# SudhirNikam/cobrix

Hardware: AMD Instinct MI355X
Metric: decoded input GB/s + records/s, fixed-len COMP-3 mix, 1-8 MI355X; % HBM peak (higher is better)
Workload: dtype u8; 1 GPU; SYN200: fixed-length 200-byte EBCDIC records, numeric mix (COMP, COMP-3, zoned DISPLAY overpunch, IBM COMP-2, cp037 X(18)) -- BASELINE config C2; records_per_gpu=50000000, input_bytes_per_gpu=10000000000, job_input_bytes=10000000000, output_columns=28, parallelism=dp1, string_layout=Arrow string views (16 B views + long payloads, one pass), occurs_layout=Arrow lists (present elements only), inputs_resident_in_hbm=True

## Files before the change

cobrix_amd/csrc/cbx_capi.hip:

```cpp
#include <hip/hip_runtime.h>

#include <algorithm>
#include <cstdio>
#include <cstring>
#include <functional>
#include <string>
#include <vector>

#include "cbx_kernels.hip"
#include "cbx_select.h"
#include "cbx_text.h"
#include "cbx_hier.h"
#include "cbx_walk.h"
#include "cbx_chain.h"
#include "cbx_filter.h"
#include "cbx_aggregate.h"
#include "cbx_group.h"
#include "cbx_topn.h"
#include "cbx_keyset.h"
#include "cbx_gather.h"

using namespace cbx;

static thread_local std::string g_err;
// ... 44 lines not shown
    bool view = false;
    bool packed = false;
    std::vector<int32_t> segid_cols;
    std::vector<ListOp> lops;
    ListOp* d_lops = nullptr;
    int32_t* d_list_len = nullptr;  int64_t list_len_cap = 0;
    int32_t* d_list_flag = nullptr; int64_t list_flag_cap = 0;
    Field* d_fields = nullptr;
    DeferSeq* d_defer = nullptr;
    uint64_t* d_defer_bits = nullptr;
    int64_t defer_bits_cap = 0;
    cbx_array* d_arrays = nullptr;
    cbx_segment_map* d_segmap = nullptr;
    uint32_t* d_lut = nullptr;
    DevColumn* d_cols = nullptr;
    std::vector<DevColumn> h_cols;
    std::vector<NumCall> h_ncall;
    std::vector<StrCall> h_scall;
    NumCall* d_ncall = nullptr;
    StrCall* d_scall = nullptr;
    size_t ncall_cap = 0, scall_cap = 0;
    std::vector<int32_t> seq_field, seq_slot;
    std::vector<int64_t> seq_tile_cap;
    std::vector<SeqCall> h_seqcall;
    std::vector<int64_t> h_seq_scratch;
    SeqCall* d_seqcall = nullptr;
    uint32_t* d_str_tot = nullptr;  int64_t str_tot_cap = 0;
    int64_t* d_str_excl = nullptr;  int64_t str_excl_cap = 0;
    int64_t* d_block_sums = nullptr; int64_t block_sums_cap = 0;
    uint32_t* d_local = nullptr;    int64_t local_cap = 0;
    uint8_t* d_scratch = nullptr;   int64_t scratch_cap = 0;
    uint64_t* d_stamps = nullptr;
    int64_t jit_min = 262144;
    bool jit_tried[4 * kPre + 5] = {};
    hipFunction_t jit_fn[4 * kPre + 5] = {};
    bool jit_coop[4 * kPre + 5] = {};
    int rec_extent = 0;
    std::string jit_error;
    int last_kind = 0;
    cbx_launch_info last_info{};
    cbx_walk_info last_walk{};
    int32_t* d_status = nullptr;
    int num_cus = 256;
    bool walk = false;
    int32_t walk_root = 0, walk_var = 0, walk_n_handlers = 0, walk_depth = 1, walk_max_rec = 0;
    cbx_walk_node* d_wnodes = nullptr;
    std::vector<cbx_walk_node> h_wnodes;
    std::vector<cbx_walk_array> h_warr;
    bool walk_jit_tried = false;
    hipFunction_t walk_jit_fn = nullptr;
    bool chain_jit_tried = false;
    hipFunction_t chain_jit_fn[5] = {};
    bool last_chain_jit = false;
    cbx_walk_array* d_warr = nullptr;
    cbx_walk_handler* d_whand = nullptr;
    int64_t* d_wslot_base = nullptr;
    int64_t* d_wtile_bytes = nullptr;
    const int64_t* d_rec_base = nullptr;
    const int32_t* d_odo = nullptr;
    int64_t odo_pitch = 0;
    const int64_t* d_dep_seed = nullptr;
    int64_t seed_pitch = 0;
    int32_t seed_root = -1;
    int64_t n_str_slots = 0;
    uint32_t* d_wcursor = nullptr; int64_t wcursor_cap = 0;
    int64_t* d_wvbase = nullptr;
    int32_t* d_wvcol = nullptr;
    int32_t* d_wvslot = nullptr;
    int32_t n_vslots = 0;
// ... 509 lines not shown

static int jit_pro(const cbx_plan* P) { return (P->opts.has_segments ? 1 : 0) | (P->harrays.empty() ? 0 : 2); }

static int launch(cbx_plan* P, const CallShape& c, const cbx_column* columns, int mode, hipStream_t st) {
    const int64_t n_tiles = (c.n_rec + kWave - 1) / kWave;
    KernelArgs a{};
    uintptr_t addr = (uintptr_t)c.data;
    a.base_shift = (int64_t)(addr & 15);
    a.data = (const uint8_t*)(addr & ~(uintptr_t)15);
    a.data_len = c.data_len + a.base_shift;
    a.rec_off = c.rec_off;
    a.rec_len = c.rec_len;
    a.n_rec = c.n_rec;
    a.n_tiles = n_tiles;
    a.pitch = n_tiles * kWave;
    a.stride = c.stride;
    a.start_off = c.start_off;
    a.first_record_id = c.first_record_id;
    a.rec_id_base = P->d_rec_base;
    a.rec_id = c.rec_id;
    a.rec_seg = c.rec_seg;
    a.odo_count = P->d_odo;
    a.odo_pitch = P->odo_pitch;
    a.file_id = c.file_id >= 0 ? c.file_id : P->opts.file_id;
    a.mode = mode;
    a.str_view = str_layout_of(P);
    const int sdw = c.stride / 4;
    const bool contig = !c.rec_off && P->contig_ok && c.stride > 0 && c.stride % 4 == 0 && a.base_shift % 4 == 0 &&
                        contig_kp(sdw) <= kPre;
    a.contig = contig ? 1 : 0;
    const int span_ext = c.start_off + P->rec_extent;
    const int span_kp = (int)std::min<int64_t>(kPre, ((int64_t)kWave * (span_ext + 8) + 32 + 1023) / 1024);
    hipFunction_t span_fn = nullptr;
    if (c.rec_off && !c.rec_id && !c.rec_seg && P->contig_ok && mode == 0 && P->jit_min >= 0 && c.n_rec >= P->jit_min &&
        (int64_t)kWave * span_ext <= 16 * 1024 && !getenv("CBX_NO_SPAN")) {
        const int k = kPre + 1 + span_kp;
        if (!P->jit_tried[k]) {
            P->jit_tried[k] = true;
            P->jit_fn[k] = jit_get(jit_source(true, span_kp, jit_pro(P), str_layout_of(P), P->cset.win, P->cset.nops, P->cset.batches,
                                              P->cset.sops, true), &P->jit_error);
        }
        span_fn = P->jit_fn[k];
    }
    const bool span = span_fn != nullptr;
    const cbx_plan::OpSet& S = (contig || span) ? P->cset : P->wset;
    if (span) {
        a.span_ext = span_ext;
        const int nch = (P->rec_extent + 15 + 15) >> 4;
        a.span_pitch = 16 * nch + 4;
        a.lds_rows = kGuard + std::max(span_kp * 1024 + 64, kWave * a.span_pitch) + kGuard;
    } else if (contig) {
        a.stride_dw = sdw;
        const int g = std::__gcd(sdw, 32);
        a.cpitch = 4 * ((g >= 4 || (g == 2 && getenv("CBX_PAD_ROWS"))) ? ((sdw & 1) ? sdw : sdw + 1) : sdw);
        a.inv_stride_dw = 1.0f / (float)sdw;
        a.lds_rows = kGuard + kWave * a.cpitch + 16 + kGuard;
    } else {
        a.lds_rows = kGuard + kWave * std::max(P->max_pitch, 16) + kGuard;
    }
    a.windows = (const CBX_CONST Window*)S.d_win;
    a.n_windows = (int)S.win.size();
    a.nops = (const CBX_CONST NumOp*)S.d_nops;
    a.batches = (const CBX_CONST Batch*)S.d_batches;
    a.sops = (const CBX_CONST StrOp*)S.d_sops;
    a.gops = (const CBX_CONST GenOp*)S.d_gops;
    a.lds_rows = (a.lds_rows + 15) & ~15;
    a.lds_counts = ((int)P->harrays.size() * kWave * 4 + 15) & ~15;
    a.str_stage = S.max_str_items > 0 ? (P->view && mode == 0 && P->view_staged ? std::max(P->str_stage, 16 * kWave) : P->str_stage) : 0;
    const int lds_base = a.lds_rows + a.lds_counts + a.str_stage;
    auto lds_blocks = [](int per_wave) {
        return (160 * 1024) / (kLutLds + kWavesPerBlock * ((per_wave + 15) & ~15));
    };
    const bool lane_dump = a.str_stage > 0 && lds_blocks(lds_base + 4 * kWave) >= lds_blocks(lds_base + 16);
    a.dump_stride = lane_dump ? 4 : 0;
    a.lds_wave = (lds_base + (lane_dump ? 4 * kWave : 16) + 15) & ~15;
    a.fields = (const CBX_CONST Field*)P->d_fields;
    a.arrays = (const CBX_CONST cbx_array*)P->d_arrays;
    a.n_arrays = (int)P->harrays.size();
    a.seg_col = P->seg_col;
    a.segmap = P->opts.has_segments ? (const CBX_CONST cbx_segment_map*)P->d_segmap : nullptr;
    a.lut = P->d_lut;
    a.cols = (const CBX_CONST DevColumn*)P->d_cols;
    a.n_seq = P->n_seq;
    a.status = P->d_status;
#ifdef CBX_STAMPS
    if (!P->d_stamps) {
        HIP_CHECK(hipMalloc((void**)&P->d_stamps, 8 * sizeof(uint64_t)));
        HIP_CHECK(hipMemset(P->d_stamps, 0, 8 * sizeof(uint64_t)));
// ... 101 lines not shown
            HIP_CHECK(hipMalloc((void**)&P->d_ncall, sizeof(NumCall) * P->h_ncall.size()));
            P->ncall_cap = P->h_ncall.size();
        }
        if (P->h_scall.size() > P->scall_cap) {
            HIP_CHECK(hipStreamSynchronize(st));
            (void)hipFree(P->d_scall);
            P->d_scall = nullptr;
            HIP_CHECK(hipMalloc((void**)&P->d_scall, sizeof(StrCall) * P->h_scall.size()));
            P->scall_cap = P->h_scall.size();
        }
        if (!P->h_ncall.empty())
            HIP_CHECK(hipMemcpyAsync(P->d_ncall, P->h_ncall.data(), sizeof(NumCall) * P->h_ncall.size(), hipMemcpyHostToDevice, st));
        if (!P->h_scall.empty())
            HIP_CHECK(hipMemcpyAsync(P->d_scall, P->h_scall.data(), sizeof(StrCall) * P->h_scall.size(), hipMemcpyHostToDevice, st));
    }
    a.ncall = (const CBX_CONST NumCall*)P->d_ncall;
    a.scall = (const CBX_CONST StrCall*)P->d_scall;
    int r;
    if (P->n_seq > 0 && (r = grow(&P->d_str_tot, &P->str_tot_cap, (int64_t)P->n_seq * n_tiles, st))) return r;
    a.str_tot = P->d_str_tot;
    const bool lists = mode == 0 && !P->lops.empty();
    if (lists && ((r = grow(&P->d_list_len, &P->list_len_cap, (int64_t)P->harrays.size() * a.pitch, st)) ||
                  (r = grow(&P->d_list_flag, &P->list_flag_cap, n_tiles, st))))
        return r;
    a.list_len = P->d_list_len;
    a.list_flag = P->d_list_flag;
    const int n_defer = n_defer_seq;
    a.defer_bits = P->d_defer_bits;
    const size_t lds_own = kLutLds + (size_t)kWavesPerBlock * a.lds_wave;
    if (lds_own > 160 * 1024) return fail(CBX_E_UNSUPPORTED, "record window does not fit in LDS");
    hipFunction_t jfn = span_fn;
    int jk = -1;
    if (!span && mode == 0 && P->jit_min >= 0 && c.n_rec >= P->jit_min) {
        const int k = contig ? contig_kp(sdw) : 0;
        if (!P->jit_tried[k]) {
            P->jit_tried[k] = true;
            size_t elems = S.sops.size();
            for (const NumOp& o : S.nops) elems += o.run > 1 ? o.run : 1;
            if (elems > (size_t)kJitMaxOps || S.win.size() > (size_t)kJitMaxWindows)
                P->jit_error = "layout has " + std::to_string(elems) + " elements in " + std::to_string(S.win.size()) +
                               " windows, above the specialised-kernel limits (" + std::to_string(kJitMaxOps) + ", " +
                               std::to_string(kJitMaxWindows) + ")";
            else {
                CoopSplit cs;
                P->jit_coop[k] = jit_coop_of(contig, span, jit_pro(P), str_layout_of(P), S.win, S.nops, S.batches, S.sops, false, &cs);
                P->jit_fn[k] = jit_get(jit_source(contig, k, jit_pro(P), str_layout_of(P), S.win, S.nops, S.batches, S.sops, false), &P->jit_error);
            }
        }
        jfn = P->jit_fn[k];
        jk = k;
    }
    P->last_kind = jfn ? 1 : 0;
    const bool coop = jfn && jk >= 0 && P->jit_coop[jk];
    const size_t lds = coop ? kLutLds + (size_t)a.lds_rows + (size_t)kWavesPerBlock * (a.lds_wave - a.lds_rows) : lds_own;
    if (lds > 160 * 1024) return fail(CBX_E_UNSUPPORTED, "record window does not fit in LDS");
    int blocks_per_cu = (int)std::max<size_t>(1, std::min<size_t>(16, (160 * 1024) / lds));
    int occ = 0;
    const hipError_t oe = jfn ? hipModuleOccupancyMaxActiveBlocksPerMultiprocessor(&occ, jfn, kWave * kWavesPerBlock, lds)
                              : hipOccupancyMaxActiveBlocksPerMultiprocessor(&occ, decode_kernel, kWave * kWavesPerBlock, lds);
    if (oe == hipSuccess && occ > 0) blocks_per_cu = std::min(blocks_per_cu, occ);
    if (!coop && contig && S.sops.size() >= S.nops.size() && S.sops.size() > 0) blocks_per_cu = std::min(blocks_per_cu, 4);
    if (const char* e = getenv("CBX_MAX_BLOCKS_PER_CU")) blocks_per_cu = std::max(1, std::min(blocks_per_cu, atoi(e)));
    const bool piped = P->pipe_peer && mode == 0 && P->packed && P->n_seq > 0;
    if (piped && P->pipe_decode_bpc > 0) blocks_per_cu = std::min(blocks_per_cu, P->pipe_decode_bpc);
    const int64_t blocks_needed = coop ? n_tiles : (n_tiles + kWavesPerBlock - 1) / kWavesPerBlock;
    const int64_t grid = std::min<int64_t>(blocks_needed, (int64_t)P->num_cus * blocks_per_cu);
    const bool prof = P->profiling && mode == 0;
    cbx_plan::CallEvents ce{{nullptr, nullptr, nullptr}};
    if (piped && P->pipe_peer->pipe_done) HIP_CHECK(hipStreamWaitEvent(st, P->pipe_peer->pipe_done, 0));
    if (prof) {
        for (auto& e : ce.e) if (!(e = take_event(P))) return fail(CBX_E_HIP, "hipEventCreate failed");
        HIP_CHECK(hipEventRecord(ce.e[0], st));
    }
    hipFunction_t cfn = nullptr;
    int ck = 0;
    if (mode == 0 && P->packed && P->n_seq > 0 && (contig || span) && P->jit_min >= 0 && c.n_rec >= P->jit_min) {
        const int kp = contig ? contig_kp(sdw) : span_kp;
        const int k = (contig ? 2 : 3) * (kPre + 1) + kp;
        if (!P->jit_tried[k]) {
            P->jit_tried[k] = true;
            std::string err;
            CoopSplit cs;
            P->jit_coop[k] = jit_coop_of(true, span, jit_pro(P), 2, S.win, S.nops, S.batches, S.sops, true, &cs);
            P->jit_fn[k] = jit_get(jit_source(true, kp, jit_pro(P), 2, S.win, S.nops, S.batches, S.sops, span, true),
                                   &err, "cbx_jit_count");
        }
        cfn = P->jit_fn[k];
        ck = k;
    }
    if (mode == 0 && P->packed && P->n_seq > 0 && !cfn && !contig) {
        const int kind = P->last_kind;
        if ((r = launch(P, c, columns, 1, st))) return r;
        P->last_kind = kind;
        if (piped) HIP_CHECK(hipEventRecord(P->pipe_done, st));
    } else if (mode == 0 && P->packed && P->n_seq > 0) {
        KernelArgs ac = a;
        ac.mode = 1;
        size_t clds = lds_own;
        const bool ccoop = cfn && P->jit_coop[ck];
        if (cfn) {
            ac.lds_wave = (a.lds_rows + a.lds_counts + 16 + 15) & ~15;
            clds = 1024 + kLutLds + (ccoop ? (size_t)a.lds_rows + (size_t)kWavesPerBlock * (ac.lds_wave - a.lds_rows)
                                           : (size_t)kWavesPerBlock * ac.lds_wave);
        }
        int cocc = 0;
        const hipError_t ce2 = cfn ? hipModuleOccupancyMaxActiveBlocksPerMultiprocessor(&cocc, cfn, kWave * kWavesPerBlock, clds)
                                   : hipOccupancyMaxActiveBlocksPerMultiprocessor(&cocc, decode_kernel, kWave * kWavesPerBlock, clds);
        int cbpc = (int)std::max<size_t>(1, std::min<size_t>(16, (160 * 1024) / clds));
        if (ce2 == hipSuccess && cocc > 0) cbpc = std::min(cbpc, cocc);
        if (const char* e = getenv("CBX_MAX_BLOCKS_PER_CU")) cbpc = std::max(1, std::min(cbpc, atoi(e)));
        if (piped && P->pipe_count_bpc > 0) cbpc = std::min(cbpc, P->pipe_count_bpc);
        const int64_t cneeded = ccoop ? n_tiles : (n_tiles + kWavesPerBlock - 1) / kWavesPerBlock;
        const int64_t cgrid = std::min<int64_t>(cneeded, (int64_t)P->num_cus * cbpc);
        if (cfn) {
            void* kargs[] = {&ac};
            HIP_CHECK(hipModuleLaunchKernel(cfn, (unsigned)cgrid, 1, 1, kWave * kWavesPerBlock, 1, 1, (unsigned)clds, st, kargs, nullptr));
        } else {
            hipLaunchKernelGGL(decode_kernel, dim3((unsigned)cgrid), dim3(kWave * kWavesPerBlock), clds, st, ac);
            HIP_CHECK(hipGetLastError());
        }
        if ((r = string_scan(P, n_tiles, st))) return r;
        if (piped) HIP_CHECK(hipEventRecord(P->pipe_done, st));
    }
    if (mode == 0) {
        cbx_launch_info li{};
        li.kind = P->last_kind;
        li.staging = span ? 2 : contig ? 1 : 0;
        li.coop = coop ? 1 : 0;
        li.kp = contig ? contig_kp(sdw) : span ? span_kp : 0;
        li.padded_rows = contig && a.cpitch != c.stride ? 1 : 0;
        li.n_windows = (int32_t)S.win.size();
        for (const Window& w : S.win)
            if (w.global && (w.nop_end > w.nop_begin || w.sop_end > w.sop_begin)) li.global_window = 1;
        li.count_kernel = !(P->packed && P->n_seq > 0) ? 0 : cfn ? 1 : 2;
        li.base_shift = (int32_t)a.base_shift;
        li.grid = grid;
        li.blocks_needed = blocks_needed;
        P->last_info = li;
    }
    if (jfn) {
        void* kargs[] = {&a};
        HIP_CHECK(hipModuleLaunchKernel(jfn, (unsigned)grid, 1, 1, kWave * kWavesPerBlock, 1, 1, (unsigned)lds, st, kargs, nullptr));
    } else {
        hipLaunchKernelGGL(decode_kernel, dim3((unsigned)grid), dim3(kWave * kWavesPerBlock), lds, st, a);
        HIP_CHECK(hipGetLastError());
    }
    if (lists) {
        const int64_t lgrid = std::min<int64_t>((n_tiles + kListWaves - 1) / kListWaves, (int64_t)P->num_cus * 8);
        const size_t llds = kListWaves * 2 * (2 * kGuard + kListStage);
        hipFunction_t lfn = nullptr;
        if (P->jit_min >= 0 && c.n_rec >= P->jit_min) {
            const int k = 4 * (kPre + 1);
            if (!P->jit_tried[k]) {
                P->jit_tried[k] = true;
                const std::string src = jit_list_source(P->lops);
                std::string err;
                if (!src.empty()) P->jit_fn[k] = jit_get(src, &err, "cbx_jit_list");
            }
            lfn = P->jit_fn[k];
        }
        const CBX_CONST ListOp* d_lops = (const CBX_CONST ListOp*)P->d_lops;
        int32_t n_lops = (int32_t)P->lops.size();
        if (lfn) {
            void* kargs[] = {&a, &d_lops, &n_lops};
            HIP_CHECK(hipModuleLaunchKernel(lfn, (unsigned)lgrid, 1, 1, kWave * kListWaves, 1, 1, (unsigned)llds, st, kargs, nullptr));
        } else {
            hipLaunchKernelGGL(list_kernel<false>, dim3((unsigned)lgrid), dim3(kWave * kListWaves), llds, st, a, d_lops, n_lops);
        }
// ... 2527 lines not shown
```

cobrix_amd/csrc/cbx_device.h:

```cpp
#pragma once
#ifndef __HIPCC_RTC__
#include <hip/hip_runtime.h>
#endif

#include "cbx_internal.h"

#ifndef CBX_DIAG
#define CBX_DIAG 0
#endif

namespace cbx {

__device__ __forceinline__ uint32_t wave_excl_scan32(uint32_t x, int lane, uint32_t& total) {
    uint32_t v = x;
    v += (uint32_t)__builtin_amdgcn_update_dpp(0, (int)v, 0x111, 0xF, 0xF, true);
    v += (uint32_t)__builtin_amdgcn_update_dpp(0, (int)v, 0x112, 0xF, 0xF, true);
    v += (uint32_t)__builtin_amdgcn_update_dpp(0, (int)v, 0x114, 0xF, 0xF, true);
    v += (uint32_t)__builtin_amdgcn_update_dpp(0, (int)v, 0x118, 0xF, 0xF, true);
    const uint32_t r0 = (uint32_t)__builtin_amdgcn_readlane((int)v, 15);
    const uint32_t r1 = (uint32_t)__builtin_amdgcn_readlane((int)v, 31);
    const uint32_t r2 = (uint32_t)__builtin_amdgcn_readlane((int)v, 47);
    const uint32_t r3 = (uint32_t)__builtin_amdgcn_readlane((int)v, 63);
    const int row = lane >> 4;
    v += (row >= 1 ? r0 : 0u) + (row >= 2 ? r1 : 0u) + (row >= 3 ? r2 : 0u);
// ... 1452 lines not shown

__device__ __forceinline__ ContigSpan contig_span(const KernelArgs& a, int64_t tile) {
    ContigSpan sp;
    const int64_t t0b = a.base_shift + tile * kWave * (int64_t)a.stride;
    const int64_t left = a.n_rec - tile * kWave;
    const int nrec_tile = left < kWave ? (left > 0 ? (int)left : 0) : kWave;
    sp.a0 = t0b & ~(int64_t)15;
    sp.mis_dw = (int)((t0b - sp.a0) >> 2);
    sp.span_dw = nrec_tile * a.stride_dw;
    sp.nch = (sp.mis_dw + sp.span_dw + 3) >> 2;
    return sp;
}

template <int KP>
__device__ __forceinline__ void contig_issue(const KernelArgs& a, const ContigSpan& sp, int lane, uint4 (&buf)[KP]) {
    int64_t left = (a.data_len - sp.a0 + 3) & ~(int64_t)3;
    left = left < 0 ? 0 : (left > (1 << 20) ? (1 << 20) : left);
    const uint64_t base = (uint64_t)(a.data + sp.a0);
    const uint32_t lo = __builtin_amdgcn_readfirstlane((uint32_t)base);
    const uint32_t hi = __builtin_amdgcn_readfirstlane((uint32_t)(base >> 32));
    const int nbytes = __builtin_amdgcn_readfirstlane((int)left);
    const int nch = __builtin_amdgcn_readfirstlane(sp.nch);
    void* bp = (void*)(((uint64_t)hi << 32) | lo);
    const __amdgpu_buffer_rsrc_t rs = __builtin_amdgcn_make_buffer_rsrc(bp, (short)0, nbytes, 0x00020000);
#pragma unroll
    for (int u = 0; u < KP; u++) {
        const int c = u * kWave + lane;
        const int off = c < nch ? 16 * c : 0x7ffffff0;
        const auto v = __builtin_amdgcn_raw_buffer_load_b128(rs, off, 0, kStageCpol);
        buf[u] = make_uint4(v[0], v[1], v[2], v[3]);
    }
}

__device__ __forceinline__ void contig_put(const KernelArgs& a, const ContigSpan& sp, int c, uint4 v, uint8_t* s_img) {
    if (a.cpitch == 4 * a.stride_dw) {
        *(uint4*)(s_img + 16 * c) = v;
        return;
    }
    uint32_t* img32 = (uint32_t*)s_img;
    const uint32_t wv[4] = {v.x, v.y, v.z, v.w};
#pragma unroll
    for (int k = 0; k < 4; k++) {
        const int d = 4 * c + k - sp.mis_dw;
        if (d >= 0 && d < sp.span_dw) {
            const int r = (int)(((float)d + 0.5f) * a.inv_stride_dw);
            img32[d + sp.mis_dw + r] = wv[k];
        }
    }
}

template <int KP>
__device__ __forceinline__ void contig_store(const KernelArgs& a, const ContigSpan& sp, int lane, const uint4 (&buf)[KP],
                                             uint8_t* s_img) {
    asm volatile("" : "+v"(lane));
#pragma unroll
    for (int u = 0; u < KP; u++) {
        const int c = u * kWave + lane;
        if (u * kWave < sp.nch && c < sp.nch) contig_put(a, sp, c, buf[u], s_img);
    }
}

__device__ __forceinline__ uint32_t stage_window(const KernelArgs& a, const Window& w, const TileCtx& t,
                                                 uint8_t* s_img, int lane) {
    const int W = w.hi - w.lo;
    const int pitch = w.pitch;
    const int nch = (W + 15 + 15) >> 4;
    const float inv_nch = 1.0f / (float)nch;
    const int64_t my_g = t.base + a.start_off + w.lo;
// ... 187 lines not shown

template <int KP, int kPro, bool kLate, typename Body>
__device__ __forceinline__ void contig_loop(const KernelArgs& a, const WaveLds& l, int64_t tile, int64_t tstep,
                                            int lane, Body body) {
    uint4 buf[KP];
    tile = first_tile<Body>(tile);
    if (tile < a.n_tiles) contig_issue<KP>(a, contig_span(a, tile), lane, buf);
    Stamps st;
    st.init();
    while (tile < a.n_tiles) {
        const ContigSpan sp = contig_span(a, tile);
        contig_store<KP>(a, sp, lane, buf, l.img);
        wave_sync_lds();
        st.mark(0);
        const int64_t next = next_tile<Body>(tile, tstep);
        body.begin(tile);
        if (!kLate) contig_issue<KP>(a, contig_span(a, next), lane, buf);
        st.mark(1);
        TileCtx t = tile_ctx<false>(a, tile, lane);
        const uint32_t rec0 = (uint32_t)(lane * a.cpitch + 4 * sp.mis_dw);
        tile_prologue<false, (kPro & 1) != 0, (kPro & 2) != 0>(a, t, l.img + rec0, lane, l.lut, l.cnt);
        st.mark(2);
        body.pre(a, t, (const uint8_t*)l.img, rec0 + (uint32_t)a.start_off, l, lane, st);
        if (kLate) contig_issue<KP>(a, contig_span(a, next), lane, buf);
        body.post(a, t, (const uint8_t*)l.img, rec0 + (uint32_t)a.start_off, l, lane, st);
        run_end(a, body, tile, lane);
        wave_sync_lds();
        st.mark(5);
        tile = next;
    }
    st.flush(a, lane);
}

template <int KP>
__device__ __forceinline__ void coop_issue(const KernelArgs& a, const ContigSpan& sp, int wid, int lane,
                                           uint4 (&buf)[(KP + kWavesPerBlock - 1) / kWavesPerBlock]) {
    constexpr int KH = (KP + kWavesPerBlock - 1) / kWavesPerBlock;
    int64_t left = a.data_len - sp.a0;
    left = left < 0 ? 0 : (left > (1 << 20) ? (1 << 20) : left);
    const uint64_t base = (uint64_t)(a.data + sp.a0);
    const uint32_t lo = __builtin_amdgcn_readfirstlane((uint32_t)base);
    const uint32_t hi = __builtin_amdgcn_readfirstlane((uint32_t)(base >> 32));
    const int nbytes = __builtin_amdgcn_readfirstlane((int)left);
    const int nch = __builtin_amdgcn_readfirstlane(sp.nch);
    void* bp = (void*)(((uint64_t)hi << 32) | lo);
    const __amdgpu_buffer_rsrc_t rs = __builtin_amdgcn_make_buffer_rsrc(bp, (short)0, nbytes, 0x00020000);
#pragma unroll
    for (int v = 0; v < KH; v++) {
        const int c = (v * kWavesPerBlock + wid) * kWave + lane;
        const int off = c < nch ? 16 * c : 0x7ffffff0;
        const auto x = __builtin_amdgcn_raw_buffer_load_b128(rs, off, 0, kStageCpol);
        buf[v] = make_uint4(x[0], x[1], x[2], x[3]);
    }
}

template <int KP>
__device__ __forceinline__ void coop_put(const KernelArgs& a, const ContigSpan& sp, int wid, int lane,
                                         const uint4 (&buf)[(KP + kWavesPerBlock - 1) / kWavesPerBlock], uint8_t* s_img) {
    constexpr int KH = (KP + kWavesPerBlock - 1) / kWavesPerBlock;
    int ln = lane;
    asm volatile("" : "+v"(ln));
#pragma unroll
    for (int v = 0; v < KH; v++) {
        const int c = (v * kWavesPerBlock + wid) * kWave + ln;
        if (c < sp.nch) contig_put(a, sp, c, buf[v], s_img);
    }
}

template <int KP, int kW, typename Body>
__device__ __forceinline__ void coop_loop(const KernelArgs& a, const WaveLds& l, int64_t tile, int64_t tstep,
                                          int lane, Body body) {
    constexpr int KH = (KP + kWavesPerBlock - 1) / kWavesPerBlock;
    uint4 buf[KH];
    constexpr int wid = kW;
    body.wid = wid;
#ifndef CBX_NO_COOP_PRIO
    if (wid == 1) __builtin_amdgcn_s_setprio(1);
#endif
    tile = first_tile<Body>(tile);
    if (tile >= a.n_tiles) return;
    coop_issue<KP>(a, contig_span(a, tile), wid, lane, buf);
    coop_put<KP>(a, contig_span(a, tile), wid, lane, buf, l.img);
    Stamps st;
    st.init();
    while (true) {
        __syncthreads();
        st.mark(0);
        const ContigSpan sp = contig_span(a, tile);
        const int64_t next = next_tile<Body>(tile, tstep);
        body.begin(tile);
        coop_issue<KP>(a, contig_span(a, next), wid, lane, buf);
        st.mark(1);
        TileCtx t = tile_ctx<false>(a, tile, lane);
        const uint32_t rec0 = (uint32_t)(lane * a.cpitch + 4 * sp.mis_dw);
        st.mark(2);
        body.template part<kW>(a, t, (const uint8_t*)l.img, rec0 + (uint32_t)a.start_off, l, lane, st);
        run_end(a, body, tile, lane);
        __syncthreads();
        st.mark(5);
        tile = next;
        if (tile >= a.n_tiles) break;
        coop_put<KP>(a, contig_span(a, tile), wid, lane, buf, l.img);
    }
    st.flush(a, lane);
}

__device__ __forceinline__ void span_recs(const KernelArgs& a, int64_t tile, int lane, int64_t& off, int32_t& len) {
    const int64_t r = tile * kWave + lane;
    const int64_t rc = r < a.n_rec ? r : a.n_rec - 1;
    const int64_t o = a.rec_off[rc];
    const int32_t l = a.rec_len[rc];
    off = a.base_shift + o;
    len = r < a.n_rec ? l : 0;
}

__device__ __forceinline__ int64_t wave_min64(int64_t v) {
#pragma unroll
    for (int m = 1; m < kWave; m <<= 1) {
        const int64_t o = __shfl_xor(v, m, kWave);
        v = o < v ? o : v;
    }
    return v;
}
__device__ __forceinline__ int64_t wave_max64(int64_t v) {
#pragma unroll
    for (int m = 1; m < kWave; m <<= 1) {
        const int64_t o = __shfl_xor(v, m, kWave);
        v = o > v ? o : v;
    }
    return v;
}

template <int KP>
__device__ __forceinline__ ContigSpan span_of(const KernelArgs& a, int64_t tile, int64_t off, int32_t len) {
    const int64_t lo = wave_min64(off);
// ... 81 lines not shown
```

cobrix_amd/csrc/cbx_jit.h:

```cpp
#pragma once
#include <hip/hiprtc.h>

#include <algorithm>
#include <cstdlib>
#include <map>
#include <mutex>
#include <sstream>
#include <string>
#include <utility>
#include <vector>

#include "cbx_jit_src.inc"

namespace cbx {

constexpr int kJitMaxStrUnroll = 16;

static std::string jit_u64(uint64_t v) {
    std::ostringstream o;
    o << "0x" << std::hex << v << "ull";
    return o.str();
}

static void jit_numop(std::ostringstream& o, const NumOp& n) {
// ... 179 lines not shown
    out->sop_mid = m_best <= ns ? sb + m_best : se;
    out->nop_mid = m_best <= ns ? 0 : m_best - ns;
    const int nnum = (int)nops.size();
    int n_defer = 0;
    for (const NumOp& op : nops) n_defer = std::max(n_defer, op.defer + 1);
    out->own[0] = out->own[1] = 0;
    for (int i = 0; i < nnum && n_words > 0; i++) {
        const int w = i < out->nop_mid ? 0 : 1;
        out->own[w] |= 1ull << i;
        if (nops[i].defer >= 0) out->own[w] |= 1ull << (nnum + nops[i].defer);
    }
    for (int i = sb; i < se && i - sb < n_str_words; i++) out->own[i < out->sop_mid ? 0 : 1] |= 1ull << (nnum + n_defer + i);
    return true;
}

static int jit_words(int layout, const std::vector<NumOp>& nops, const std::vector<Batch>& batches,
                     const std::vector<StrOp>& sops, bool span, bool count, int* n_str_words) {
    int n_defer = 0;
    bool runs = false;
    for (const NumOp& op : nops) n_defer = std::max(n_defer, op.defer + 1);
    for (const Batch& b : batches) runs |= b.runs != 0;
    *n_str_words = layout == 1 && getenv("CBX_STR_VWORDS") ? (int)sops.size() : 0;
    return (count || runs || span || getenv("CBX_NO_VWORDS")) ? 0 : (int)nops.size() + n_defer + *n_str_words;
}

static bool jit_coop_of(bool contig, bool span, int pro, int layout, const std::vector<Window>& win, const std::vector<NumOp>& nops,
                        const std::vector<Batch>& batches, const std::vector<StrOp>& sops, bool count, CoopSplit* out) {
    int nsw = 0;
    const int nw = contig ? jit_words(layout, nops, batches, sops, span, count, &nsw) : 0;
    return jit_coop(contig, span, pro, win, nops, batches, sops, count, nw, nsw, out);
}

static std::string jit_source(bool contig, int kp, int pro, int layout, const std::vector<Window>& win, const std::vector<NumOp>& nops,
                              const std::vector<Batch>& batches, const std::vector<StrOp>& sops, bool span, bool count = false) {
    std::ostringstream o;
    const bool view = layout == 1;
    if (const char* d = getenv("CBX_JIT_DEFINES")) {
        std::string s(d);
        for (size_t b = 0; b < s.size();) {
            size_t e = s.find(',', b);
            if (e == std::string::npos) e = s.size();
            std::string m = s.substr(b, e - b);
            const size_t q = m.find('=');
            if (!m.empty()) o << "#define " << (q == std::string::npos ? m : m.substr(0, q) + " " + m.substr(q + 1)) << "\n";
            b = e + 1;
        }
    }
    if (getenv("CBX_STR_NO_SHIFT")) o << "#define CBX_STR_NO_SHIFT 1\n";
    o << "#define CBX_STR_LAYOUT " << layout << "\n";
    o << "#define CBX_MODE " << (count ? 1 : 0) << "\n";
    if (count) o << "#define CBX_COUNT_LUT 1\n";
    o << "#include \"cbx_device.h\"\n";
    bool late = !count && contig && !sops.empty() && (!nops.empty() || win.size() > 1);
    if (const char* e = getenv("CBX_JIT_LATE")) late = late && e[0] != '0';
    CoopSplit cs;
    const bool coop = jit_coop_of(contig, span, pro, layout, win, nops, batches, sops, count, &cs);
    if (contig) {
        int n_defer = 0;
        for (const NumOp& op : nops) n_defer = std::max(n_defer, op.defer + 1);
        int n_str_words = 0;
        const int n_words = jit_words(layout, nops, batches, sops, span, count, &n_str_words);
        const int nv = std::max(1, (n_words + 7) / 8);
        const char* sig = "(const KernelArgs& a, const TileCtx& t, const uint8_t* img,\n"
                          "      uint32_t rec_addr, const WaveLds& l, int lane, Stamps& st) {\n";
        o << "namespace cbx {\n"
             "struct JitBody {\n"
             "  static constexpr int kWords = " << n_words << ";\n"
             "  int wid = 0;   // (coop_loop: the wave's part of the tile)\n";
        if (n_words > 0) o << "  VWords<" << nv << ", " << nops.size() << ", " << n_defer << "> vw;\n";
        else o << "  DirectSink vw;\n";
        if (n_words > 0 && coop)
            o << "  __device__ __forceinline__ void begin(int64_t tile) { vw.j = (int)(tile % kVRun); }\n"
                 "  __device__ __forceinline__ void flush(const KernelArgs& a, int64_t t0, int lane) { vw.flush(a, kWords, t0, lane, wid ? "
              << jit_u64(cs.own[1]) << " : " << jit_u64(cs.own[0]) << "); }\n";
        else
            o << (n_words > 0 ? "  __device__ __forceinline__ void begin(int64_t tile) { vw.j = (int)(tile % kVRun); }\n"
                                  "  __device__ __forceinline__ void flush(const KernelArgs& a, int64_t t0, int lane) { vw.flush(a, kWords, t0, lane); }\n"
                                : "  __device__ __forceinline__ void begin(int64_t) {}\n"
                                  "  __device__ __forceinline__ void flush(const KernelArgs&, int64_t, int) {}\n");
        if (coop) {
            std::vector<Window> wa(win), wb(win);
            wa[0].sop_end = cs.sop_mid;
            wb[0].sop_begin = cs.sop_mid;
            o << "  template <int kW>\n  __device__ __forceinline__ void part" << sig
              << "    if constexpr (kW == 0) {\n";
            jit_window_ops(o, wa, 0, nops, batches, sops, true, layout, 1, count, true);
            if (!count) jit_window_ops(o, win, 0, nops, batches, sops, true, layout, 2, count, true, 0, cs.nop_mid, false);
            o << "    } else {\n";
            jit_window_ops(o, wb, 0, nops, batches, sops, true, layout, 1, count, true);
// ... 199 lines not shown
    if (const char* d = getenv("CBX_JIT_DUMP")) {
        if (g_jit_cache.find(std::make_pair(dev, src)) == g_jit_cache.end()) {
            const std::string path = std::string(d) + "/" + name + "_" + std::to_string(g_jit_cache.size()) + ".hip";
            if (FILE* f = fopen(path.c_str(), "w")) {
                fwrite(src.data(), 1, src.size(), f);
                fclose(f);
            }
        }
    }
    auto key = std::make_pair(dev, src);
    auto it = g_jit_cache.find(key);
    if (it == g_jit_cache.end()) {
        JitKernel k;
        std::vector<char> code;
        if (jit_compile(src, &code, &k.error) && hipModuleLoadData(&k.module, code.data()) != hipSuccess) {
            k.module = nullptr;
            k.error = "hipModuleLoadData failed for the specialised kernel";
        }
        it = g_jit_cache.emplace(key, k).first;
    }
    JitKernel& k = it->second;
    *err = k.error;
    if (!k.module) return nullptr;
    auto f = k.fns.find(name);
    if (f == k.fns.end()) {
        hipFunction_t fn = nullptr;
        if (hipModuleGetFunction(&fn, k.module, name) != hipSuccess) fn = nullptr;
        f = k.fns.emplace(name, fn).first;
    }
    if (!f->second) *err = std::string("hipModuleGetFunction failed for ") + name;
    return f->second;
}

}
```

cobrix_amd/native.py:

```python
from __future__ import annotations

import ctypes
import os

_HERE = os.path.dirname(os.path.abspath(__file__))
LIB_PATH = os.path.join(_HERE, "libcobrix_hip_%s.so" % os.environ["CBX_LIB_VARIANT"]
                        if os.environ.get("CBX_LIB_VARIANT") else "libcobrix_hip.so")

CBX_MAX_DIMS = 4
CBX_MAX_SEG_KEYS = 32
CBX_MAX_SEG_KEY_LEN = 32
CBX_MAX_SEG_LEVELS = 8
CBX_MAX_SEG_PREFIX = 64

K_STRING, K_STRING_ASCII, K_HEX, K_RAW, K_BCD, K_BINARY, K_ZONED = 1, 2, 3, 4, 5, 6, 7
K_ASCII_NUM, K_UTF16_BE, K_UTF16_LE = 8, 13, 14
K_FLOAT, K_DOUBLE, K_RECORD_ID, K_FILE_ID = 9, 10, 11, 12
O_I32, O_I64, O_DEC64, O_DEC128, O_F32, O_F64, O_STRING, O_BINARY = 1, 2, 3, 4, 5, 6, 7, 8
F_SIGNED, F_BIG_ENDIAN, F_EXPLICIT_DOT, F_INTEGRAL, F_IBM, F_LITTLE_ENDIAN_FP, F_DEPENDEE = (
    0x1, 0x2, 0x4, 0x8, 0x10, 0x20, 0x40)
F_LIST = 0x80
TRIM = {"none": 1, "left": 2, "right": 3, "both": 4}

CBX_OK, CBX_E_ARGUMENT, CBX_E_STATE, CBX_E_CAPACITY, CBX_E_HIP, CBX_E_UNSUPPORTED = 0, -1, -2, -3, -4, -5
# ... 234 lines not shown


CBX_HIER_MAX_SEG, CBX_HIER_MAX_EVENTS, CBX_HIER_MAX_DEPS = 16, 32, 16
HIER_EVENT_END = -32768


class CbxHierDependee(ctypes.Structure):
    _fields_ = [("values", ctypes.c_void_p), ("validity", ctypes.c_void_p), ("out_type", ctypes.c_int32),
                ("walk_slot", ctypes.c_int32)]


class CbxHierOdoArray(ctypes.Structure):
    _fields_ = [("dependee", ctypes.c_int32), ("out_row", ctypes.c_int32), ("min_count", ctypes.c_int32),
                ("max_count", ctypes.c_int32), ("first_counts", ctypes.c_void_p)]


class CbxHierWalk(ctypes.Structure):
    _fields_ = [("n_segments", ctypes.c_int32), ("root_segment", ctypes.c_int32),
                ("table_base", ctypes.c_int64 * (CBX_HIER_MAX_SEG + 1)),
                ("table_rows", ctypes.c_int64 * (CBX_HIER_MAX_SEG + 1)),
                ("child_offsets", ctypes.c_void_p * CBX_HIER_MAX_SEG),
                ("children", (ctypes.c_int8 * CBX_HIER_MAX_SEG) * CBX_HIER_MAX_SEG),
                ("events", (ctypes.c_int16 * CBX_HIER_MAX_EVENTS) * (CBX_HIER_MAX_SEG + 1)),
                ("seeds", ctypes.c_void_p)]


STAGING_WINDOWED, STAGING_CONTIGUOUS, STAGING_SPAN = 0, 1, 2


class CbxLaunchInfo(ctypes.Structure):
    _fields_ = [(n, ctypes.c_int32) for n in ("kind", "staging", "coop", "kp", "padded_rows", "n_windows",
                                                "global_window", "count_kernel", "base_shift", "reserved")] + \
               [("grid", ctypes.c_int64), ("blocks_needed", ctypes.c_int64)]


def launch_info(plan_handle) -> CbxLaunchInfo:
    info = CbxLaunchInfo()
    check(load().cbx_plan_launch_info(plan_handle, ctypes.byref(info)))
    return info


class CbxWalkInfo(ctypes.Structure):
    _fields_ = [(n, ctypes.c_int32) for n in ("kind", "stage_cap", "vlds", "wave_lds", "depth", "stack_lds",
                                                "n_vslots", "n_sslots")] + \
               [("grid", ctypes.c_int64), ("n_tiles", ctypes.c_int64)]


def walk_info(plan_handle) -> CbxWalkInfo:
    info = CbxWalkInfo()
    check(load().cbx_plan_walk_info(plan_handle, ctypes.byref(info)))
    return info


_lib = None


def lib_path() -> str:
    return LIB_PATH


def load():
    global _lib
    if _lib is not None:
        return _lib
    if not os.path.exists(LIB_PATH):
        raise NativeLibraryError(f"{LIB_PATH} is missing: run __graft_entry__.build() (hipcc --offload-arch=gfx950)")
# ... 87 lines not shown
```

include/cobrix_hip.h:

```cpp
#ifndef COBRIX_HIP_H
#define COBRIX_HIP_H
#ifndef __HIPCC_RTC__
#include <stdint.h>
#else
typedef __hip_internal::int8_t int8_t;
typedef __hip_internal::uint8_t uint8_t;
typedef __hip_internal::int16_t int16_t;
typedef __hip_internal::uint16_t uint16_t;
typedef __hip_internal::int32_t int32_t;
typedef __hip_internal::uint32_t uint32_t;
typedef __hip_internal::int64_t int64_t;
typedef __hip_internal::uint64_t uint64_t;
#endif

#ifdef __cplusplus
extern "C" {
#endif

#define CBX_ABI_VERSION 25

#define CBX_OK 0
#define CBX_E_ARGUMENT (-1)
#define CBX_E_STATE (-2)
#define CBX_E_CAPACITY (-3)
// ... 129 lines not shown
                           int32_t rec_stride, int32_t start_offset, int64_t* out_sizes, void* stream);

int cbx_decode_fixed(cbx_plan* plan, const uint8_t* d_records, int64_t n_rec, int32_t rec_stride,
                     int32_t start_offset, int64_t first_record_id, cbx_column* columns, void* stream);

int cbx_decode_var(cbx_plan* plan, const uint8_t* d_data, int64_t n_bytes, const int64_t* d_rec_off,
                   const int32_t* d_rec_len, int64_t n_rec, int32_t start_offset,
                   int64_t first_record_id, cbx_column* columns, void* stream);
int cbx_string_sizes_var(cbx_plan* plan, const uint8_t* d_data, int64_t n_bytes, const int64_t* d_rec_off,
                         const int32_t* d_rec_len, int64_t n_rec, int32_t start_offset,
                         int64_t* out_sizes, void* stream);

int cbx_plan_set_record_base(cbx_plan* plan, const int64_t* d_base);

int cbx_plan_set_odo_counts(cbx_plan* plan, const int32_t* d_counts, int64_t pitch);

int cbx_plan_check(cbx_plan* plan, void* stream);

int cbx_plan_set_profiling(cbx_plan* plan, int32_t enable);
int cbx_plan_kernel_times(cbx_plan* plan, float* decode_ms, float* post_ms, int32_t max_calls, int32_t* n_calls);

int cbx_plan_kernel_kind(cbx_plan* plan, int32_t* kind);

typedef struct cbx_launch_info {
    int32_t kind;
    int32_t staging;
    int32_t coop;
    int32_t kp;
    int32_t padded_rows;
    int32_t n_windows;
    int32_t global_window;
    int32_t count_kernel;
    int32_t base_shift;
    int32_t reserved;
    int64_t grid, blocks_needed;
} cbx_launch_info;
int cbx_plan_launch_info(cbx_plan* plan, cbx_launch_info* out);

typedef struct cbx_walk_info {
    int32_t kind;
    int32_t stage_cap;
    int32_t vlds;
    int32_t wave_lds;
    int32_t depth;
    int32_t stack_lds;
    int32_t n_vslots;
    int32_t n_sslots;
    int64_t grid, n_tiles;
} cbx_walk_info;
int cbx_plan_walk_info(cbx_plan* plan, cbx_walk_info* out);

int cbx_plan_direct_eligible(const cbx_plan* plan, int32_t* eligible);

int cbx_plan_frame_kind(cbx_plan* plan, int32_t* kind);

int cbx_plan_specialize(cbx_plan* plan, char* source, int64_t source_cap, int64_t* source_len, int32_t compile);

typedef struct {
    int32_t big_endian;
    int32_t adjustment;
    int32_t file_header_bytes;
    int32_t file_footer_bytes;
} cbx_rdw_params;

int cbx_frame_rdw(const uint8_t* d_data, int64_t n_bytes, const int64_t* seeds, int32_t n_seeds,
                  const cbx_rdw_params* params, int64_t* d_rec_off, int32_t* d_rec_len,
                  int64_t capacity, int64_t* n_records, void* stream);
// ... 323 lines not shown
```

Baseline: 2655 GB/s.

## Specialise cooperative staging on padded-row flag with precomputed buffer offsets

The JIT now bakes whether contiguous LDS rows are padded into the kernel via CBX_ROWS_PADDED and caches padded and unpadded variants in separate slots. In the cooperative staging path, the wave index becomes a template parameter. Per-chunk bounds checks are replaced by a buffer resource clamped to the exact span, with offsets precomputed and held in place by scheduling barriers. Unpadded rows take a direct linear LDS store. The change also reports kernel scratch bytes through launch info, so register spills can be seen; this adds more JIT variants and relies on buffer out-of-range behaviour for the tail.

```diff
diff --git a/cobrix_amd/csrc/cbx_capi.hip b/cobrix_amd/csrc/cbx_capi.hip
--- a/cobrix_amd/csrc/cbx_capi.hip
+++ b/cobrix_amd/csrc/cbx_capi.hip
@@ -100,9 +100,11 @@
     uint8_t* d_scratch = nullptr;   int64_t scratch_cap = 0;
     uint64_t* d_stamps = nullptr;
     int64_t jit_min = 262144;
-    bool jit_tried[4 * kPre + 5] = {};
-    hipFunction_t jit_fn[4 * kPre + 5] = {};
-    bool jit_coop[4 * kPre + 5] = {};
+    static constexpr int kJitPadSlot = 4 * kPre + 5;
+    bool jit_tried[2 * kJitPadSlot] = {};
+    hipFunction_t jit_fn[2 * kJitPadSlot] = {};
+    bool jit_coop[2 * kJitPadSlot] = {};
+    int32_t jit_scratch[2 * kJitPadSlot] = {};
     int rec_extent = 0;
     std::string jit_error;
     int last_kind = 0;
@@ -678,6 +680,7 @@
     const int span_ext = c.start_off + P->rec_extent;
     const int span_kp = (int)std::min<int64_t>(kPre, ((int64_t)kWave * (span_ext + 8) + 32 + 1023) / 1024);
     hipFunction_t span_fn = nullptr;
+    int span_slot = -1;
     if (c.rec_off && !c.rec_id && !c.rec_seg && P->contig_ok && mode == 0 && P->jit_min >= 0 && c.n_rec >= P->jit_min &&
         (int64_t)kWave * span_ext <= 16 * 1024 && !getenv("CBX_NO_SPAN")) {
         const int k = kPre + 1 + span_kp;
@@ -685,11 +688,14 @@
             P->jit_tried[k] = true;
             P->jit_fn[k] = jit_get(jit_source(true, span_kp, jit_pro(P), str_layout_of(P), P->cset.win, P->cset.nops, P->cset.batches,
                                               P->cset.sops, true), &P->jit_error);
+            P->jit_scratch[k] = jit_scratch_bytes(P->jit_fn[k]);
         }
         span_fn = P->jit_fn[k];
+        span_slot = k;
     }
     const bool span = span_fn != nullptr;
     const cbx_plan::OpSet& S = (contig || span) ? P->cset : P->wset;
+    bool padded = false;
     if (span) {
         a.span_ext = span_ext;
         const int nch = (P->rec_extent + 15 + 15) >> 4;
@@ -700,6 +706,7 @@
         const int g = std::__gcd(sdw, 32);
         a.cpitch = 4 * ((g >= 4 || (g == 2 && getenv("CBX_PAD_ROWS"))) ? ((sdw & 1) ? sdw : sdw + 1) : sdw);
         a.inv_stride_dw = 1.0f / (float)sdw;
+        padded = a.cpitch != c.stride;
         a.lds_rows = kGuard + kWave * a.cpitch + 16 + kGuard;
     } else {
         a.lds_rows = kGuard + kWave * std::max(P->max_pitch, 16) + kGuard;
@@ -867,7 +874,8 @@
     hipFunction_t jfn = span_fn;
     int jk = -1;
     if (!span && mode == 0 && P->jit_min >= 0 && c.n_rec >= P->jit_min) {
-        const int k = contig ? contig_kp(sdw) : 0;
+        const int kp = contig ? contig_kp(sdw) : 0;
+        const int k = kp + (padded ? cbx_plan::kJitPadSlot : 0);
         if (!P->jit_tried[k]) {
             P->jit_tried[k] = true;
             size_t elems = S.sops.size();
@@ -879,7 +887,9 @@
             else {
                 CoopSplit cs;
                 P->jit_coop[k] = jit_coop_of(contig, span, jit_pro(P), str_layout_of(P), S.win, S.nops, S.batches, S.sops, false, &cs);
-                P->jit_fn[k] = jit_get(jit_source(contig, k, jit_pro(P), str_layout_of(P), S.win, S.nops, S.batches, S.sops, false), &P->jit_error);
+                P->jit_fn[k] = jit_get(jit_source(contig, kp, jit_pro(P), str_layout_of(P), S.win, S.nops, S.batches, S.sops, false, false,
+                                                  contig ? (int)padded : -1), &P->jit_error);
+                P->jit_scratch[k] = jit_scratch_bytes(P->jit_fn[k]);
             }
         }
         jfn = P->jit_fn[k];
@@ -911,14 +921,14 @@
     int ck = 0;
     if (mode == 0 && P->packed && P->n_seq > 0 && (contig || span) && P->jit_min >= 0 && c.n_rec >= P->jit_min) {
         const int kp = contig ? contig_kp(sdw) : span_kp;
-        const int k = (contig ? 2 : 3) * (kPre + 1) + kp;
+        const int k = (contig ? 2 : 3) * (kPre + 1) + kp + (padded ? cbx_plan::kJitPadSlot : 0);
         if (!P->jit_tried[k]) {
             P->jit_tried[k] = true;
             std::string err;
             CoopSplit cs;
             P->jit_coop[k] = jit_coop_of(true, span, jit_pro(P), 2, S.win, S.nops, S.batches, S.sops, true, &cs);
-            P->jit_fn[k] = jit_get(jit_source(true, kp, jit_pro(P), 2, S.win, S.nops, S.batches, S.sops, span, true),
-                                   &err, "cbx_jit_count");
+            P->jit_fn[k] = jit_get(jit_source(true, kp, jit_pro(P), 2, S.win, S.nops, S.batches, S.sops, span, true,
+                                              contig ? (int)padded : -1), &err, "cbx_jit_count");
         }
         cfn = P->jit_fn[k];
         ck = k;
@@ -963,12 +973,13 @@
         li.staging = span ? 2 : contig ? 1 : 0;
         li.coop = coop ? 1 : 0;
         li.kp = contig ? contig_kp(sdw) : span ? span_kp : 0;
-        li.padded_rows = contig && a.cpitch != c.stride ? 1 : 0;
+        li.padded_rows = padded ? 1 : 0;
         li.n_windows = (int32_t)S.win.size();
         for (const Window& w : S.win)
             if (w.global && (w.nop_end > w.nop_begin || w.sop_end > w.sop_begin)) li.global_window = 1;
         li.count_kernel = !(P->packed && P->n_seq > 0) ? 0 : cfn ? 1 : 2;
         li.base_shift = (int32_t)a.base_shift;
+        li.scratch_bytes = !jfn ? 0 : P->jit_scratch[jk >= 0 ? jk : span_slot];
         li.grid = grid;
         li.blocks_needed = blocks_needed;
         P->last_info = li;
diff --git a/cobrix_amd/csrc/cbx_device.h b/cobrix_amd/csrc/cbx_device.h
--- a/cobrix_amd/csrc/cbx_device.h
+++ b/cobrix_amd/csrc/cbx_device.h
@@ -1508,8 +1508,27 @@
     }
 }
 
+__device__ __forceinline__ bool rows_padded(const KernelArgs& a) {
+#ifdef CBX_ROWS_PADDED
+    (void)a;
+    return CBX_ROWS_PADDED != 0;
+#else
+    return a.cpitch != 4 * a.stride_dw;
+#endif
+}
+#ifdef CBX_ROWS_PADDED
+constexpr bool kCoopExact = true;
+#else
+constexpr bool kCoopExact = false;
+#endif
+#if defined(CBX_ROWS_PADDED) && !defined(CBX_COOP_TEST_ROWS)
+constexpr bool kRowsLinear = CBX_ROWS_PADDED == 0;
+#else
+constexpr bool kRowsLinear = false;
+#endif
+
 __device__ __forceinline__ void contig_put(const KernelArgs& a, const ContigSpan& sp, int c, uint4 v, uint8_t* s_img) {
-    if (a.cpitch == 4 * a.stride_dw) {
+    if (!rows_padded(a)) {
         *(uint4*)(s_img + 16 * c) = v;
         return;
     }
@@ -1763,37 +1782,90 @@
     st.flush(a, lane);
 }
 
-template <int KP>
-__device__ __forceinline__ void coop_issue(const KernelArgs& a, const ContigSpan& sp, int wid, int lane,
+template <int KP, int kW>
+__device__ __forceinline__ void coop_issue(const KernelArgs& a, const ContigSpan& sp, int lane,
                                            uint4 (&buf)[(KP + kWavesPerBlock - 1) / kWavesPerBlock]) {
     constexpr int KH = (KP + kWavesPerBlock - 1) / kWavesPerBlock;
+    static_assert(KP <= kPre, "chunk offsets stay below 16 KiB");
+    if constexpr (!kCoopExact) {
+        int64_t left = a.data_len - sp.a0;
+        left = left < 0 ? 0 : (left > (1 << 20) ? (1 << 20) : left);
+        const uint64_t base = (uint64_t)(a.data + sp.a0);
+        const uint32_t lo = __builtin_amdgcn_readfirstlane((uint32_t)base);
+        const uint32_t hi = __builtin_amdgcn_readfirstlane((uint32_t)(base >> 32));
+        const int nbytes = __builtin_amdgcn_readfirstlane((int)left);
+        const int nch = __builtin_amdgcn_readfirstlane(sp.nch);
+        void* bp = (void*)(((uint64_t)hi << 32) | lo);
+        const __amdgpu_buffer_rsrc_t rs = __builtin_amdgcn_make_buffer_rsrc(bp, (short)0, nbytes, 0x00020000);
+#pragma unroll
+        for (int v = 0; v < KH; v++) {
+            const int c = (v * kWavesPerBlock + kW) * kWave + lane;
+            const int off = c < nch ? 16 * c : 0x7ffffff0;
+            const auto x = __builtin_amdgcn_raw_buffer_load_b128(rs, off, 0, kStageCpol);
+            buf[v] = make_uint4(x[0], x[1], x[2], x[3]);
+        }
+        return;
+    }
     int64_t left = a.data_len - sp.a0;
-    left = left < 0 ? 0 : (left > (1 << 20) ? (1 << 20) : left);
+    const int64_t span = 16 * (int64_t)sp.nch;
+    left = left < 0 ? 0 : (left > span ? span : left);
     const uint64_t base = (uint64_t)(a.data + sp.a0);
     const uint32_t lo = __builtin_amdgcn_readfirstlane((uint32_t)base);
     const uint32_t hi = __builtin_amdgcn_readfirstlane((uint32_t)(base >> 32));
     const int nbytes = __builtin_amdgcn_readfirstlane((int)left);
-    const int nch = __builtin_amdgcn_readfirstlane(sp.nch);
     void* bp = (void*)(((uint64_t)hi << 32) | lo);
     const __amdgpu_buffer_rsrc_t rs = __builtin_amdgcn_make_buffer_rsrc(bp, (short)0, nbytes, 0x00020000);
+    int ln = lane;
+#ifndef CBX_COOP_HOIST
+    asm volatile("" : "+v"(ln));
+#endif
+    int vo[(KP + 3) / 4];
+#pragma unroll
+    for (int k = 0; k < (KP + 3) / 4; k++) {
+        vo[k] = 16 * ln + 4096 * k;
+#ifndef CBX_COOP_SPREAD
+        asm volatile("" : "+v"(vo[k]));
+#endif
+    }
+#ifndef CBX_COOP_SPREAD
+    __builtin_amdgcn_sched_barrier(0);
+#endif
 #pragma unroll
     for (int v = 0; v < KH; v++) {
-        const int c = (v * kWavesPerBlock + wid) * kWave + lane;
-        const int off = c < nch ? 16 * c : 0x7ffffff0;
-        const auto x = __builtin_amdgcn_raw_buffer_load_b128(rs, off, 0, kStageCpol);
+        const int row = v * kWavesPerBlock + kW;
+        if (row >= KP) continue;
+        const auto x = __builtin_amdgcn_raw_buffer_load_b128(rs, vo[row / 4] + 1024 * (row % 4), 0, kStageCpol);
         buf[v] = make_uint4(x[0], x[1], x[2], x[3]);
     }
-}
-
-template <int KP>
-__device__ __forceinline__ void coop_put(const KernelArgs& a, const ContigSpan& sp, int wid, int lane,
+#ifndef CBX_COOP_SPREAD
+    __builtin_amdgcn_sched_barrier(0);
+#endif
+}
+
+template <int KP, int kW>
+__device__ __forceinline__ void coop_put(const KernelArgs& a, const ContigSpan& sp, int lane,
                                          const uint4 (&buf)[(KP + kWavesPerBlock - 1) / kWavesPerBlock], uint8_t* s_img) {
     constexpr int KH = (KP + kWavesPerBlock - 1) / kWavesPerBlock;
     int ln = lane;
     asm volatile("" : "+v"(ln));
+    if constexpr (!kCoopExact) {
+#pragma unroll
+        for (int v = 0; v < KH; v++) {
+            const int c = (v * kWavesPerBlock + kW) * kWave + ln;
+            if (c < sp.nch) contig_put(a, sp, c, buf[v], s_img);
+        }
+        return;
+    }
 #pragma unroll
     for (int v = 0; v < KH; v++) {
-        const int c = (v * kWavesPerBlock + wid) * kWave + ln;
+        const int row = v * kWavesPerBlock + kW;
+        if (row >= KP) continue;
+        const int c = row * kWave + ln;
+        if (kRowsLinear && row < KP - 1) {
+            *(uint4*)(s_img + 16 * c) = buf[v];
+            continue;
+        }
+        asm volatile("" ::"v"(buf[v].x), "v"(buf[v].y), "v"(buf[v].z), "v"(buf[v].w));
         if (c < sp.nch) contig_put(a, sp, c, buf[v], s_img);
     }
 }
@@ -1810,8 +1882,8 @@
 #endif
     tile = first_tile<Body>(tile);
     if (tile >= a.n_tiles) return;
-    coop_issue<KP>(a, contig_span(a, tile), wid, lane, buf);
-    coop_put<KP>(a, contig_span(a, tile), wid, lane, buf, l.img);
+    coop_issue<KP, kW>(a, contig_span(a, tile), lane, buf);
+    coop_put<KP, kW>(a, contig_span(a, tile), lane, buf, l.img);
     Stamps st;
     st.init();
     while (true) {
@@ -1820,7 +1892,7 @@
         const ContigSpan sp = contig_span(a, tile);
         const int64_t next = next_tile<Body>(tile, tstep);
         body.begin(tile);
-        coop_issue<KP>(a, contig_span(a, next), wid, lane, buf);
+        coop_issue<KP, kW>(a, contig_span(a, next), lane, buf);
         st.mark(1);
         TileCtx t = tile_ctx<false>(a, tile, lane);
         const uint32_t rec0 = (uint32_t)(lane * a.cpitch + 4 * sp.mis_dw);
@@ -1831,7 +1903,7 @@
         st.mark(5);
         tile = next;
         if (tile >= a.n_tiles) break;
-        coop_put<KP>(a, contig_span(a, tile), wid, lane, buf, l.img);
+        coop_put<KP, kW>(a, contig_span(a, tile), lane, buf, l.img);
     }
     st.flush(a, lane);
 }
diff --git a/cobrix_amd/csrc/cbx_jit.h b/cobrix_amd/csrc/cbx_jit.h
--- a/cobrix_amd/csrc/cbx_jit.h
+++ b/cobrix_amd/csrc/cbx_jit.h
@@ -235,7 +235,8 @@
 }
 
 static std::string jit_source(bool contig, int kp, int pro, int layout, const std::vector<Window>& win, const std::vector<NumOp>& nops,
-                              const std::vector<Batch>& batches, const std::vector<StrOp>& sops, bool span, bool count = false) {
+                              const std::vector<Batch>& batches, const std::vector<StrOp>& sops, bool span, bool count = false,
+                              int padded = -1) {
     std::ostringstream o;
     const bool view = layout == 1;
     if (const char* d = getenv("CBX_JIT_DEFINES")) {
@@ -249,15 +250,17 @@
             b = e + 1;
         }
     }
+    CoopSplit cs;
+    const bool coop = jit_coop_of(contig, span, pro, layout, win, nops, batches, sops, count, &cs);
+    const bool exact = coop && !count && !nops.empty() && padded >= 0;
     if (getenv("CBX_STR_NO_SHIFT")) o << "#define CBX_STR_NO_SHIFT 1\n";
     o << "#define CBX_STR_LAYOUT " << layout << "\n";
     o << "#define CBX_MODE " << (count ? 1 : 0) << "\n";
     if (count) o << "#define CBX_COUNT_LUT 1\n";
+    if (exact) o << "#define CBX_ROWS_PADDED " << (padded ? 1 : 0) << "\n";
     o << "#include \"cbx_device.h\"\n";
     bool late = !count && contig && !sops.empty() && (!nops.empty() || win.size() > 1);
     if (const char* e = getenv("CBX_JIT_LATE")) late = late && e[0] != '0';
-    CoopSplit cs;
-    const bool coop = jit_coop_of(contig, span, pro, layout, win, nops, batches, sops, count, &cs);
     if (contig) {
         int n_defer = 0;
         for (const NumOp& op : nops) n_defer = std::max(n_defer, op.defer + 1);
@@ -523,4 +526,11 @@
     return f->second;
 }
 
-}
+static int32_t jit_scratch_bytes(hipFunction_t fn) {
+    int v = 0;
+    if (!fn) return 0;
+    if (hipFuncGetAttribute(&v, HIP_FUNC_ATTRIBUTE_LOCAL_SIZE_BYTES, fn) != hipSuccess) return -1;
+    return (int32_t)v;
+}
+
+}
diff --git a/cobrix_amd/native.py b/cobrix_amd/native.py
--- a/cobrix_amd/native.py
+++ b/cobrix_amd/native.py
@@ -290,6 +290,10 @@
     _fields_ = [(n, ctypes.c_int32) for n in ("kind", "staging", "coop", "kp", "padded_rows", "n_windows",
                                                 "global_window", "count_kernel", "base_shift", "reserved")] + \
                [("grid", ctypes.c_int64), ("blocks_needed", ctypes.c_int64)]
+
+    @property
+    def scratch_bytes(self) -> int:
+        return int(self.reserved)
 
 
 def launch_info(plan_handle) -> CbxLaunchInfo:
diff --git a/include/cobrix_hip.h b/include/cobrix_hip.h
--- a/include/cobrix_hip.h
+++ b/include/cobrix_hip.h
@@ -185,7 +185,10 @@
     int32_t global_window;
     int32_t count_kernel;
     int32_t base_shift;
-    int32_t reserved;
+    union {
+        int32_t scratch_bytes;
+        int32_t reserved;
+    };
     int64_t grid, blocks_needed;
 } cbx_launch_info;
 int cbx_plan_launch_info(cbx_plan* plan, cbx_launch_info* out);
```

Measured after the change: 2682 GB/s, median of 5. No clear change (+1.0%).
